# drscotthawley/signaltrain

Hardware: AMD Instinct MI355X
Metric: audio-frames/sec (train step) comp_4c 8192-sample windows @ 1/2/4/8 GPUs (higher is better)
Workload: dtype f32; 1 GPU; comp_4c synthetic, 8192-sample windows, batch 256/GPU, fp32 (BASELINE configs[1]); window=8192, frames_per_window=25, global_batch=256, parallelism=dp1

## Files before the change

### signaltrain_amd/csrc/st_ae.h

```cpp
#pragma once
#include "st_common.h"

namespace sta {

constexpr int NL = 9;
#ifndef ST_AE_ABLATE
#define ST_AE_ABLATE 0
#endif

struct AEOffsets { int w[NL]; int b[NL]; };

struct GroupWalk { int first, end, stride; };
__device__ __forceinline__ GroupWalk fwd_group_walk(const int ngroups, const int NW, const int wave)
{
    const int G = (int)gridDim.x, b = (int)blockIdx.x;
    if ((G & 7) == 0) {
        const int S = G >> 3, x = b & 7, slot = b >> 3;
        const int per = (ngroups + 7) >> 3;
        const int lo = x * per, hi = lo + per < ngroups ? lo + per : ngroups;
        return GroupWalk{lo + wave * S + slot, hi, S * NW};
    }
    return GroupWalk{wave * G + b, ngroups, G * NW};
}

// ... 108 lines not shown
                                   const int tid, const int l0, const int l1, const bool dgrad_images)
{
    const float* const nets[1] = {ae};
    ae_load_nets<NT, BF, 1>(lds, CL::tab(), nets, go, T, OT, K, tid, l0, l1, dgrad_images, true);
}
template <int NT, int BF = 0>
__device__ inline void ae_load_lds2(float* lds, const float* __restrict__ ae_m, const float* __restrict__ ae_p, const AEOffsets& go,
                                    const int T, const int OT, const int K, const int tid, const int l0, const int l1)
{
    const float* const nets[2] = {ae_m, ae_p};
    ae_load_nets<NT, BF, 2>(lds, CL::tab(), nets, go, T, OT, K, tid, l0, l1, false, true);
}

template <int NT>
__host__ __device__ __forceinline__ void ae_partials_store(float* base, const float* lds, const int stride, const AETab& tab, const AEOffsets& go,
                                                           const int PG, const int T, const int OT, const int K, const int tid, const int l0, const int l1,
                                                           const unsigned have_mask)
{
    auto sum4 = [&](int idx) { return (lds[idx] + lds[stride + idx]) + (lds[2 * stride + idx] + lds[3 * stride + idx]); };
    const AEShape sh{T, OT, K};
#pragma unroll
    for (int l = 0; l < NL; ++l) {
        if (l < l0 || l >= l1) continue;
        const bool have = (have_mask >> l) & 1;
        const int IN = sh.in(l), n = sh.out(l) * IN;
#pragma unroll
        for (int u = 0; u < (ae_max_elems(l) + NT - 1) / NT; ++u) {
            const int e = tid + u * NT;
            if (e < n) { const int o = e / IN, i = e - o * IN; base[go.w[l] + e] = have ? sum4(tab.ao[l] + o * ae_inp(l) + i) : 0.f; }
        }
        if (tid < sh.out(l)) base[go.b[l] + tid] = have ? sum4(tab.bo[l] + tid) : 0.f;
        { const int p0 = go.w[l] + n, np = go.b[l] - p0; if (tid < np) base[p0 + tid] = 0.f; }
        { const int p0 = go.b[l] + sh.out(l), np = (l + 1 < NL ? go.w[l + 1] : PG) - p0; if (tid < np) base[p0 + tid] = 0.f; }
    }
}

constexpr int AE_IMG_DG = CL::BWD_TOTAL - CL::FWD_TOTAL;
__host__ __device__ constexpr int ae_img_fwd_floats(const int FP) { return 2 * CL::FWD_TOTAL + FP; }
__host__ __device__ constexpr int ae_img_floats(const int FP) { return ae_img_fwd_floats(FP) + 2 * AE_IMG_DG; }
struct AEImgJob { const float* ae[2]; float* img; AEOffsets go; int T, OT, K, F, FP; float expfac; int n, n_blk; };
__host__ __device__ __forceinline__ float ae_freq_weight(const float expfac, const int f) { return expf(expfac * (float)f); }
__host__ __device__ __forceinline__ void ae_img_build(const AEImgJob& j, const int p)
{
    if (p >= j.n) return;
    const AEShape sh{j.T, j.OT, j.K};
    constexpr AETab tab = CL::tab();
    float v = 0.f;
    const int q0 = p - 2 * CL::FWD_TOTAL;
    if (q0 >= 0 && q0 < j.FP) v = q0 < j.F ? ae_freq_weight(j.expfac, q0) : 0.f;
    else {
        const bool dg = q0 >= 0;
        const int net = dg ? (q0 - j.FP >= AE_IMG_DG) : (p >= CL::FWD_TOTAL);
        const int q = dg ? q0 - j.FP - net * AE_IMG_DG : p - net * CL::FWD_TOTAL;
        const float* __restrict__ ae = j.ae[net];
        if (!dg && q >= CL::AEND) {
#pragma unroll
            for (int l = 0; l < NL; ++l)
                if (q >= tab.bo[l] && q < tab.bo[l] + ae_outp(l)) { const int o = q - tab.bo[l]; if (o < sh.out(l)) v = ae[j.go.b[l] + o]; }
        } else {
#pragma unroll
            for (int l = 0; l < NL; ++l)
                if (q >= tab.ao[l] && q < tab.ao[l] + ae_max_elems(l)) {
                    const int s = (q - tab.ao[l]) >> 2, lo = (q - tab.ao[l]) & 3;
                    const int o = dg ? ((s / ae_inp(l)) << 2) + lo : s % ae_outp(l);
                    const int i = dg ? s % ae_inp(l) : ((s / ae_outp(l)) << 2) + lo;
                    if (o < sh.out(l) && i < sh.in(l)) v = ae[j.go.w[l] + o * sh.in(l) + i];
// ... 577 lines not shown
#pragma unroll
        for (int it = 0; it < ITL; ++it)
#pragma unroll
            for (int r = 0; r < 4; ++r) {
                float* p = dW + (16 * ot + 4 * g + r) * INP + 16 * it + c;
                if constexpr (FIRST) *p = acc[ot][it][r]; else *p += acc[ot][it][r];
            }
}
template <int OTL, bool FIRST>
__device__ __forceinline__ void db_flush(float* dst, float (&db)[OTL], const int g, const int c)
{
#pragma unroll
    for (int ot = 0; ot < OTL; ++ot) {
        float v = db[ot];
        v += __shfl_xor(v, 16); v += __shfl_xor(v, 32);
        if (g == 0) { if constexpr (FIRST) dst[16 * ot + c] = v; else dst[16 * ot + c] += v; }
    }
}

__device__ __forceinline__ void group_colsum_store(float* __restrict__ dst, const f32x4& t, const int g, const int c)
{
    const float v = (t[0] + t[1]) + (t[2] + t[3]);
    const unsigned u = __builtin_bit_cast(unsigned, v);
    const auto p = __builtin_amdgcn_permlane16_swap(u, u, false, false);
    const float w = __builtin_bit_cast(float, (unsigned)p[0]) + __builtin_bit_cast(float, (unsigned)p[1]);
    const unsigned x = __builtin_bit_cast(unsigned, w);
    const auto q = __builtin_amdgcn_permlane32_swap(x, x, false, false);
    const float s = __builtin_bit_cast(float, (unsigned)q[0]) + __builtin_bit_cast(float, (unsigned)q[1]);
    if (g == 0) dst[c] = s;
}

constexpr int AE_BWD_SCR = (32 + 16 + 16) * SP + 2 * 4 * 320;
constexpr int ae_bwd_lds_floats(int nw) { return (CL::BWD_TOTAL + nw * AE_BWD_SCR) > nw * CL::FWD_TOTAL ? (CL::BWD_TOTAL + nw * AE_BWD_SCR) : nw * CL::FWD_TOTAL; }
template <int NW, bool INNER = false, int BF = 0, int VAR = 1, bool SAVED = false, bool KG = false, bool IMG = false>
__global__ void __launch_bounds__(NW * 64, 1)
ae_bwd_kernel(const float* __restrict__ mag, const float* __restrict__ phs, const float* __restrict__ knobs,
              const float* __restrict__ ae_m, const float* __restrict__ ae_p, const AEOffsets go, const int PG,
              const float* __restrict__ mag_hat, const float* __restrict__ phs_hat, const float* __restrict__ dAA,
              const float* __restrict__ g_mag_hat, const float reg_coef, const float expfac,
              float* __restrict__ dmag, float* __restrict__ dphs, float* __restrict__ ws,
              const int B, const int T, const int OT, const int F, const int K, const int KP,
              const int to_lo, const int to_hi,
              const int nslab, const size_t slab,
              const float* __restrict__ sv = nullptr,
              float* __restrict__ kg = nullptr,
              const float* __restrict__ img = nullptr)
{
    static_assert(!SAVED || (!INNER && BF == 0), "the kept-activation backward exists for the fused fp32 geometries");
    static_assert(!IMG || SAVED, "ready-made images: the kept-activation backward only");
    extern __shared__ __attribute__((aligned(16))) float lds[];
    const int ae = blockIdx.y;
    const int tid = threadIdx.x, lane = tid & 63, wave = tid >> 6;
    const int g = lane >> 4, c = lane & 15;
    float* lw = lds;
    float* Vs = lds + CL::BWD_TOTAL + wave * AE_BWD_SCR;
    float* Ys = Vs + 32 * SP;
    float* Ts = Ys + 16 * SP;
    float* XH = Ts + 16 * SP;
    float* XD = XH + 4 * 320;
    if constexpr (IMG && !(ST_AE_ABLATE & 128)) {
        const int FPi = KP / 2;
        const float* const dg = img + 2 * CL::FWD_TOTAL + FPi + ae * AE_IMG_DG;
        constexpr int N4 = AE_IMG_DG / 4, U = (N4 + NW * 64 - 1) / (NW * 64);
        f32x4 v[U];
#pragma unroll
        for (int u = 0; u < U; ++u) { const int e = tid + u * NW * 64; v[u] = reinterpret_cast<const f32x4*>(dg)[e < N4 ? e : 0]; }
        for (int i = tid; i < FPi / 4; i += NW * 64) reinterpret_cast<f32x4*>(lds)[i] = reinterpret_cast<const f32x4*>(img + 2 * CL::FWD_TOTAL)[i];
#pragma unroll
        for (int u = 0; u < U; ++u) { const int e = tid + u * NW * 64; if (e < N4) reinterpret_cast<f32x4*>(lds + CL::G0)[e] = v[u]; }
    } else
    ae_load_lds<NW * 64, BF>(lw, ae ? ae_p : ae_m, go, INNER ? 16 : T, INNER ? 16 : OT, K, tid, INNER ? 1 : 0, INNER ? 8 : NL, true);
    __syncthreads();

    const float* vin = ae ? phs : mag;
    const float* dh8in = ae ? phs_hat : mag_hat;
    float* dvout = ae ? dphs : dmag;
    const int FP = KP / 2, gpw = FP / 16;
    const int ngroups = B * gpw;
    const int gstride = gridDim.x * NW;

    f32x4 rW1[4][2], rW2[2][4], rW3[1][2], rW4[1][1], rW5[1][2], rW6[1][1], rW7[2][1], rW8[4][2], rW9[1][4];
    float rb1[4], rb2[2], rb3[1], rb4[1], rb5[1], rb6[1], rb7[2], rb8[4], rb9[1];
// ... 52 lines not shown
        const float* const dB0 = dA0 + FP, * const dB1 = dA1 + FP, * const dB2 = dA2 + FP;
        const unsigned bOT = ST_MUL24(bq, OT), btF = ST_MUL24(ST_MUL24(bq, T), F) + (unsigned)fq;
#pragma unroll
        for (int r = 0; r < 4; ++r) {
            const int to = 4 * g + r;
            const bool ok = fvq && to < OT;
            const bool lv = ok && to >= to_lo && to <= to_hi;
            const unsigned ro = bOT + (unsigned)(ok ? to : 0);
            const unsigned p0 = ST_MUL24(lv ? ro : 0u, KP) + (unsigned)fq;
            const unsigned pF = ST_MUL24(ro, F) + (unsigned)fq;
#if ST_AE_ABLATE & 1
            q_x[r][0] = q_x[r][1] = q_x[r][2] = q_y[r][0] = q_y[r][1] = q_y[r][2] = 1e-3f * (float)(p0 & 7); q_ph[r] = 0.3f; q_mh[r] = 0.2f + 1e-3f * (float)(pF & 3);
#else
            q_x[r][0] = ldg32(dA0, p0); q_x[r][1] = ldg32(dA1, p0); q_x[r][2] = ldg32(dA2, p0);
            q_y[r][0] = ldg32(dB0, p0); q_y[r][1] = ldg32(dB1, p0); q_y[r][2] = ldg32(dB2, p0);
            q_ph[r] = ldg32(phs_hat, pF); q_mh[r] = ldg32(mag_hat, pF);
#endif
            if constexpr (GM) q_gm[r] = ldg32(g_mag_hat, pF); else q_gm[r] = 0.f;
            if constexpr (!TAIL16) q_mt[r] = ldg32(vin, btF + ST_MUL24(ok ? T - OT + to : 0, F));
        }
    };
    f32x4 s_h1[4], s_h2[2], s_h3[1], s_h4[1], s_h5[1], s_h6[1], s_h7[2], s_h8[4], s_e9[1];
    const float* const svn = SAVED ? sv + (size_t)ae * ngroups * (AE_SV_TILES * 256) : nullptr;
    const unsigned lane16 = (unsigned)lane << 4;
#ifdef ST_SV_DIAG
    auto svp = [&](const int gq) { return svn + (size_t)(__builtin_amdgcn_readfirstlane(gq) & ST_SV_DIAG) * (AE_SV_TILES * 256); };
#else
    auto svp = [&](const int gq) { return svn + (size_t)__builtin_amdgcn_readfirstlane(gq) * (AE_SV_TILES * 256); };
#endif
    if constexpr (SAVED) {
        if (grp < ngroups) {
            load_q(grp);
            const float* const p = svp(grp);
            sv_load(p, lane16, 16, s_e9); sv_load(p, lane16, 12, s_h8); sv_load(p, lane16, 10, s_h7); sv_load(p, lane16, 9, s_h6); sv_load(p, lane16, 8, s_h5);
            sv_load(p, lane16, 7, s_h4); sv_load(p, lane16, 6, s_h3); sv_load(p, lane16, 4, s_h2); sv_load(p, lane16, 0, s_h1);
        }
    }

    for (; grp < ngroups; grp += gstride) {
        asm volatile("" ::: "memory");
        const int b = grp / gpw, f = (grp - b * gpw) * 16 + c;
        const bool fv = f < F;
        if constexpr (!INNER && !SAVED) load_q(grp);
        f32x4 h1in[4], dh8[4];
        if constexpr (INNER) {
            const unsigned col0 = (unsigned)b * FP + (unsigned)(grp - b * gpw) * 16;
#pragma unroll
            for (int ot = 0; ot < 4; ++ot) {
#pragma unroll
                for (int r = 0; r < 4; ++r) {
                    h1in[ot][r] = ldg32(vin, (unsigned)(16 * ot + 4 * g + r) * Rw + col0 + c);
                    dh8[ot][r] = ldg32(dh8in, (unsigned)(16 * ot + 4 * g + r) * Rw + col0 + c);
                }
            }
        }
        f32x4 vn[2], knn; float knTn;
        const int gnext = grp + gstride < ngroups ? grp + gstride : grp;
#if ST_AE_ABLATE & 64
        vn[0] = vr[0]; vn[1] = vr[1]; knn = kn; knTn = knT;
#else
        if constexpr (!INNER) load_v(gnext, vn);
        load_kn(gnext, knn, knTn);
#endif

        f32x4 h1[4], h2[2], h3[1], h4[1], h5[1], h6[1], h7[2], h8[4], e9[1];
        f32x4 fr9[1 * 4];
        if constexpr (SAVED) {
#pragma unroll
            for (int it = 0; it < 2; ++it)
#pragma unroll
                for (int r = 0; r < 4; ++r) Vs[(16 * it + 4 * g + r) * SP + c] = vr[it][r];
#pragma unroll
            for (int k = 0; k < 4; ++k) { h1[k] = s_h1[k]; h8[k] = s_h8[k]; }
#pragma unroll
            for (int k = 0; k < 2; ++k) { h2[k] = s_h2[k]; h7[k] = s_h7[k]; }
            h3[0] = s_h3[0]; h4[0] = s_h4[0]; h5[0] = s_h5[0]; h6[0] = s_h6[0]; e9[0] = s_e9[0];
        } else {
        f32x4 fr2[2 * 4];
        if constexpr (INNER) {
#pragma unroll
            for (int ot = 0; ot < 4; ++ot) h1[ot] = h1in[ot];
            frags_fwd<2, 4, CL::O1, BF>(fr2, lw + CL::A1, g, c);
        } else {
            f32x4 fr1[4 * 2]; frags_fwd<4, 2, CL::O0, BF>(fr1, lw + CL::A0, g, c);
            frags_fwd<2, 4, CL::O1, BF>(fr2, lw + CL::A1, g, c);
#pragma unroll
            for (int it = 0; it < 2; ++it)
#pragma unroll
                for (int r = 0; r < 4; ++r) Vs[(16 * it + 4 * g + r) * SP + c] = vr[it][r];
            ST_FENCE();
            fwdD_fr<4, 2, BF>(fr1, lw + CL::B0, vr, h1, g);
        }
        f32x4 fr3[1 * 2]; frags_fwd<1, 2, CL::O2, BF>(fr3, lw + CL::A2, g, c); ST_FENCE(); fwdD_fr<2, 4, BF>(fr2, lw + CL::B1, h1, h2, g);
        f32x4 fr4[1 * 1]; frags_fwd<1, 1, CL::O3, BF>(fr4, lw + CL::A3, g, c); ST_FENCE(); fwdD_fr<1, 2, BF>(fr3, lw + CL::B2, h2, h3, g);
        f32x4 fr5[1 * 2]; frags_fwd<1, 2, CL::O4, BF>(fr5, lw + CL::A4, g, c); ST_FENCE(); fwdD_fr<1, 1, BF>(fr4, lw + CL::B3, h3, h4, g);
        f32x4 fr6[1 * 1]; frags_fwd<1, 1, CL::O5, BF>(fr6, lw + CL::A5, g, c); ST_FENCE();
        {
            const f32x4 hk[2] = {h4[0], kn};
            fwdD_fr<1, 2, BF>(fr5, lw + CL::B4, hk, h5, g);
        }
        f32x4 fr7[2 * 1]; frags_fwd<2, 1, CL::O6, BF>(fr7, lw + CL::A6, g, c); ST_FENCE(); fwdD_fr<1, 1, BF>(fr6, lw + CL::B5, h5, h6, g);
        f32x4 fr8[4 * 2]; frags_fwd<4, 2, CL::O7, BF>(fr8, lw + CL::A7, g, c); ST_FENCE(); fwdD_fr<2, 1, BF>(fr7, lw + CL::B6, h6, h7, g);
        if constexpr (!INNER) frags_fwd<1, 4, CL::O8, BF>(fr9, lw + CL::A8, g, c);
        ST_FENCE(); fwdD_fr<4, 2, BF>(fr8, lw + CL::B7, h7, h8, g);
        }
        f32x4 da9[1];
        float dxA[4], mtA[4];
        if constexpr (!INNER) {
            ST_FENCE();
// ... 6 lines not shown
                const bool ok = fv && to < OT;
                const bool lv = ok && to >= to_lo && to <= to_hi;
                const float gre = lv ? q_x[r][0] + (nslab > 1 ? q_x[r][1] : 0.f) + (nslab > 2 ? q_x[r][2] : 0.f) : 0.f;
                const float gim = lv ? q_y[r][0] + (nslab > 1 ? q_y[r][1] : 0.f) + (nslab > 2 ? q_y[r][2] : 0.f) : 0.f;
                const float ph = q_ph[r], mh = q_mh[r];
                if constexpr (!TAIL16) asm volatile("" :: "v"(q_mt[r]));
                float sn, cs; st_sincos(ph, sn, cs);
                const float sg = mh > 0.f ? 1.f : (mh < 0.f ? -1.f : 0.f);
                const float dmh = gre * cs + gim * sn + reg_coef * sg * wf + (GM ? q_gm[r] : 0.f);
                const float dph = mh * (gim * cs - gre * sn);
                dxA[r] = ok ? (ae == 0 ? dmh : dph) : 0.f;
                mtA[r] = ae == 0 ? (TAIL16 ? vr[1][r] : q_mt[r]) : 1.f;
            }
            if constexpr (!SAVED) fwdD_fr<1, 4, BF>(fr9, lw + CL::B8, h8, e9, g);
            if constexpr (BF == 0 && !SAVED) {
#pragma unroll
                for (int p_ = 0; p_ < 16; ++p_) { __builtin_amdgcn_sched_group_barrier(0x008, 1, 0); __builtin_amdgcn_sched_group_barrier(0x002, 7, 0); }
            }
            ST_FENCE();
        }
        if constexpr (!INNER) {
#pragma unroll
            for (int r = 0; r < 4; ++r) {
                const int to = 4 * g + r;
                const float eg = elu_grad_from_out(e9[0][r]);
                const float e1 = ae == 0 ? e9[0][r] : 1.f;
                const float d9 = dxA[r] * mtA[r] * eg;
                const float tail = dxA[r] * e1;
                da9[0][r] = d9;
                Ts[to * SP + c] = tail;
                Ys[to * SP + c] = d9;
            }
        }
#define ST_REFILL(...) do { if constexpr (SAVED) { ST_FENCE(); __VA_ARGS__; ST_FENCE(); } } while (0)
        const float* const svq = SAVED ? svp(gnext) : nullptr;
        ST_REFILL(load_q(gnext); sv_load(svq, lane16, 16, s_e9));
#define ST_PIPE(N_) do { \
        __builtin_amdgcn_sched_group_barrier(0x008, (N_) + 2, 0); \
        _Pragma("unroll") for (int p_ = 0; p_ < (N_) - 2; ++p_) { \
            __builtin_amdgcn_sched_group_barrier(0x002, 2, 0); __builtin_amdgcn_sched_group_barrier(0x300, 1, 0); \
            __builtin_amdgcn_sched_group_barrier(0x008, 1, 0); } \
        ST_FENCE(); } while (0)
#define ST_BWD_STAGE(O_, I_, FD_, DA_, DAT_, HP_, HTP_, DAP_, DATP_, RW_, RB_, NEXT_) \
        to_Th<I_, BF>(XH, HP_, HTP_, g, c); ST_FENCE(); \
        dgradD_fr<O_, I_, BF>(FD_, DA_, DAP_); mul_elu_grad<I_>(DAP_, HP_); \
        to_T<I_>(XD, DAP_, DATP_, g, c); NEXT_; \
        wgrad_regh<O_, I_, BF>(RW_, RB_, DAT_, HTP_); \
        ST_PIPE(BF ? O_ * I_ : O_ * I_ * 4);
        typedef typename TTy<BF>::type tt_t;
        tt_t hT8[4]; f32x4 da8[4], daT8[4], fd8[2 * 4];
        if constexpr (INNER) {
            frags_dgrad<4, 2, CL::I7, BF>(fd8, lw + CL::G7, g, c);
            to_Th<4, BF>(XH, h8, hT8, g, c);
#pragma unroll
            for (int ot = 0; ot < 4; ++ot) da8[ot] = dh8[ot];
            mul_elu_grad<4>(da8, h8); to_T<4>(XD, da8, daT8, g, c);
        } else {
            f32x4 daT9[1], fd9[4 * 1];
            frags_dgrad<1, 4, CL::I8, BF>(fd9, lw + CL::G8, g, c);
            daT9[0] = *reinterpret_cast<const f32x4*>(Ys + c * SP + 4 * g);
            ST_BWD_STAGE(1, 4, fd9, da9, daT9, h8, hT8, da8, daT8, rW9, rb9, (frags_dgrad<4, 2, CL::I7, BF>(fd8, lw + CL::G7, g, c)))
            ST_REFILL(sv_load(svq, lane16, 12, s_h8));
        }
        tt_t hT7[2]; f32x4 da7[2], daT7[2], fd7[1 * 2];
        ST_BWD_STAGE(4, 2, fd8, da8, daT8, h7, hT7, da7, daT7, rW8, rb8, (frags_dgrad<2, 1, CL::I6, BF>(fd7, lw + CL::G6, g, c)))
        ST_REFILL(sv_load(svq, lane16, 10, s_h7));
        tt_t hT6[1]; f32x4 da6[1], daT6[1], fd6[1];
        ST_BWD_STAGE(2, 1, fd7, da7, daT7, h6, hT6, da6, daT6, rW7, rb7, (frags_dgrad<1, 1, CL::I5, BF>(fd6, lw + CL::G5, g, c)))
        ST_REFILL(sv_load(svq, lane16, 9, s_h6));
        tt_t hT5[1]; f32x4 da5[1], daT5[1], fd5[1];
        ST_BWD_STAGE(1, 1, fd6, da6, daT6, h5, hT5, da5, daT5, rW6, rb6, (frags_dgrad<1, 1, CL::I4, BF>(fd5, lw + CL::G4, g, c)))
        ST_REFILL(sv_load(svq, lane16, 8, s_h5));
        tt_t hT4[1], hT4k[2]; f32x4 da4[1], daT4[1], fd4[1];
        {
            to_Th<1, BF>(XH, h4, hT4, g, c); ST_FENCE();
            dgradD_fr<1, 1, BF>(fd5, da5, da4); mul_elu_grad<1>(da4, h4);
            to_T<1>(XD, da4, daT4, g, c); frags_dgrad<1, 1, CL::I3, BF>(fd4, lw + CL::G3, g, c); ST_FENCE();
            hT4k[0] = hT4[0];
            hT4k[1] = tt_splat<BF>(knT);
            wgrad_regh<1, 2, BF>(rW5, rb5, daT5, hT4k);
            if constexpr (KG) group_colsum_store(kg + ((size_t)ae * ngroups + grp) * 16, daT5[0], g, c);
        }
        ST_REFILL(sv_load(svq, lane16, 7, s_h4));
        tt_t hT3[1]; f32x4 da3[1], daT3[1], fd3[2 * 1];
        ST_BWD_STAGE(1, 1, fd4, da4, daT4, h3, hT3, da3, daT3, rW4, rb4, (frags_dgrad<1, 2, CL::I2, BF>(fd3, lw + CL::G2, g, c)))
        ST_REFILL(sv_load(svq, lane16, 6, s_h3));
        tt_t hT2[2]; f32x4 da2[2], daT2[2], fd2[4 * 2];
        ST_BWD_STAGE(1, 2, fd3, da3, daT3, h2, hT2, da2, daT2, rW3, rb3, (frags_dgrad<2, 4, CL::I1, BF>(fd2, lw + CL::G1, g, c)))
        ST_REFILL(sv_load(svq, lane16, 4, s_h2));
        tt_t hT1[4]; f32x4 da1[4], daT1[4], fd1[2 * 4];
        if constexpr (INNER) {
            to_Th<4, BF>(XH, h1, hT1, g, c); ST_FENCE();
            dgradD_fr<2, 4, BF>(fd2, da2, da1); mul_elu_grad<4>(da1, h1);
            const unsigned col0 = (unsigned)b * FP + (unsigned)(grp - b * gpw) * 16;
#pragma unroll
            for (int ot = 0; ot < 4; ++ot)
#pragma unroll
                for (int r = 0; r < 4; ++r) stg32(dvout, (unsigned)(16 * ot + 4 * g + r) * Rw + col0 + c, da1[ot][r]);
            ST_FENCE();
            wgrad_regh<2, 4, BF>(rW2, rb2, daT2, hT1);
        } else {
            ST_BWD_STAGE(2, 4, fd2, da2, daT2, h1, hT1, da1, daT1, rW2, rb2, (frags_dgrad<4, 2, CL::I0, BF>(fd1, lw + CL::G0, g, c)))
            ST_REFILL(sv_load(svq, lane16, 0, s_h1));
        }
        f32x4 vT[2], dv[2];
        if constexpr (!INNER) {
#pragma unroll
            for (int it = 0; it < 2; ++it) vT[it] = *reinterpret_cast<const f32x4*>(Vs + (16 * it + c) * SP + 4 * g);
            ST_FENCE();
            dgradD_fr<4, 2, BF>(fd1, da1, dv);
            wgrad_reg<4, 2, BF>(rW1, rb1, daT1, vT);
        }
#undef ST_BWD_STAGE
#undef ST_PIPE
#undef ST_REFILL
        if constexpr (!INNER) {
            mask_v(gnext, vn);
            vr[0] = vn[0]; vr[1] = vn[1];
        }
        mask_kn(knn, knTn); kn = knn; knT = knTn;
        if constexpr (!INNER) {
        float dvs[2][4], tls[2][4];
#pragma unroll
        for (int it = 0; it < 2; ++it)
#pragma unroll
            for (int r = 0; r < 4; ++r) {
                dvs[it][r] = dv[it][r]; asm volatile("" : "+v"(dvs[it][r]));
                const int ti = 16 * it + 4 * g + r - (T - OT);
                tls[it][r] = Ts[(ti >= 0 && ti < OT ? ti : 0) * SP + c];
            }
        const unsigned dv0 = ST_MUL24(ST_MUL24(b, T), F) + (unsigned)f;
#pragma unroll
        for (int it = 0; it < 2; ++it)
#pragma unroll
            for (int r = 0; r < 4; ++r) {
                const int t = 16 * it + 4 * g + r;
                const float v = dvs[it][r] + (t >= T - OT ? tls[it][r] : 0.f);
#if ST_AE_ABLATE & 2
                asm volatile("" :: "v"(v));
#else
                if (fv && t < T) stg32(dvout, dv0 + ST_MUL24(t, F), v);
#endif
            }
        }
    }
#if ST_AE_ABLATE & 256
    {
#define ST_KT(x, A, Bq) { _Pragma("unroll") for (int a_ = 0; a_ < A; ++a_) _Pragma("unroll") for (int b_ = 0; b_ < Bq; ++b_) _Pragma("unroll") for (int r_ = 0; r_ < 4; ++r_) asm volatile("" :: "v"(x[a_][b_][r_])); }
#define ST_KB(x, A) { _Pragma("unroll") for (int a_ = 0; a_ < A; ++a_) asm volatile("" :: "v"(x[a_])); }
        ST_KT(rW1, 4, 2) ST_KT(rW2, 2, 4) ST_KT(rW3, 1, 2) ST_KT(rW4, 1, 1) ST_KT(rW5, 1, 2) ST_KT(rW6, 1, 1) ST_KT(rW7, 2, 1) ST_KT(rW8, 4, 2) ST_KT(rW9, 1, 4)
        ST_KB(rb1, 4) ST_KB(rb2, 2) ST_KB(rb3, 1) ST_KB(rb4, 1) ST_KB(rb5, 1) ST_KB(rb6, 1) ST_KB(rb7, 2) ST_KB(rb8, 4) ST_KB(rb9, 1)
#undef ST_KT
#undef ST_KB
        return;
    }
#endif
    __syncthreads();
    static_assert(NW == 4, "the store pass sums exactly four per-wave images");
    float* dwl = lds + wave * CL::FWD_TOTAL;
    if constexpr (!INNER) { dw_flush<4, 2, CL::I0, true>(dwl + CL::A0, rW1, g, c); dw_flush<1, 4, CL::I8, true>(dwl + CL::A8, rW9, g, c);
                            db_flush<4, true>(dwl + CL::B0, rb1, g, c); db_flush<1, true>(dwl + CL::B8, rb9, g, c); }
    dw_flush<2, 4, CL::I1, true>(dwl + CL::A1, rW2, g, c); dw_flush<1, 2, CL::I2, true>(dwl + CL::A2, rW3, g, c);
    dw_flush<1, 1, CL::I3, true>(dwl + CL::A3, rW4, g, c); dw_flush<1, 2, CL::I4, true>(dwl + CL::A4, rW5, g, c);
    dw_flush<1, 1, CL::I5, true>(dwl + CL::A5, rW6, g, c); dw_flush<2, 1, CL::I6, true>(dwl + CL::A6, rW7, g, c);
    dw_flush<4, 2, CL::I7, true>(dwl + CL::A7, rW8, g, c);
    db_flush<2, true>(dwl + CL::B1, rb2, g, c); db_flush<1, true>(dwl + CL::B2, rb3, g, c); db_flush<1, true>(dwl + CL::B3, rb4, g, c);
    db_flush<1, true>(dwl + CL::B4, rb5, g, c); db_flush<1, true>(dwl + CL::B5, rb6, g, c); db_flush<2, true>(dwl + CL::B6, rb7, g, c);
    db_flush<4, true>(dwl + CL::B7, rb8, g, c);
    __syncthreads();
    ae_partials_store<NW * 64>(ws + ((size_t)blockIdx.x * 2 + ae) * PG, lds, CL::FWD_TOTAL, CL::tab(), go, PG, T, OT, K, tid, 0, NL,
                               INNER ? 0x0FEu : 0x1FFu);
}

}
```

### signaltrain_amd/csrc/st_api.hip

```cpp
#include <hip/hip_runtime.h>
#include <stdarg.h>
#include <stdio.h>
#include <string.h>
#include <math.h>
#include <mutex>
#include <set>
#include <type_traits>
#include <utility>
#include "st_common.h"
#include "st_gemm.h"
#include "st_gemm_planes.h"
#include "st_gemm_tn.h"
#include "st_gemm16.h"
#include "st_misc.h"
#include "st_ae.h"
#include "st_ae_wide.h"
#include "st_ae_split.h"
#include "st_ae32.h"
#include "st_dp.h"
#include "st_feed.h"
#include "st_feed_files.h"

static thread_local char g_err[512] = "";
int st_fail(int code, const char* fmt, ...)
// ... 132 lines not shown
    return n;
}
extern "C" int st_set_debug(int v) { return v == 0 ? ST_OK : st_fail(ST_ERR_ARG, "st_set_debug(%d): the product library has no run-time ablations (build with -DST_*_ABLATE=bits)", v); }
static int g_dp_inline = 1;
static int g_ae_save = 1;
static int g_ae_split = -1;
static int g_ae32 = 1;
static int g_pl_bf16 = 0;
static int g_wg_split = 0;
static int g_pl_dgrad = 0;
static int g_pl_shape = 3;
static int g_g16 = 1;
static int g_g16_dma = 0;
static int g_nt128 = 1;
static int g_tn128 = 1;
static int g_tn_fm = 3;
static int g_g16_crop = 15;
static int g_frs_nt = 1;
static int g_xt = 0;
static const int NORM_E_PARTIALS = 32;
static const int NORM_E_MAX = 4096;
static int g_wide_direct = 1;
static int g_an_bk = 32;
static int g_bk = 16;
static int g_wg_mode = 0;
#define ST_TUNING_LIST(X) X(g_ae_split, -1) X(g_ae_save, 1) X(g_dp_inline, 1) X(g_pl_bf16, 0) X(g_wg_split, 0) X(g_pl_dgrad, 0) X(g_pl_shape, 3) X(g_g16, 1) X(g_g16_dma, 0) \
    X(g_nt128, 1) X(g_tn128, 1) X(g_frs_nt, 1) X(g_xt, 0) X(g_an_bk, 32) X(g_bk, 16) X(g_wg_mode, 0) X(g_ae32, 1) X(g_wide_direct, 1) X(g_tn_fm, 3) X(g_g16_crop, 15)
static const struct { int first, count; int* var; int value; int* also; } k_tuning_codes[] = {
    {16, 1, &g_an_bk, 16, &g_bk}, {32, 1, &g_an_bk, 32, &g_bk},
    {100, 1, &g_wg_mode, 0, nullptr}, {102, 1, &g_wg_mode, 2, nullptr},
    {7000, 2, &g_xt, 0, nullptr},
    {8000, 2, &g_ae_split, 0, nullptr}, {8002, 1, &g_ae_split, -1, nullptr},
    {8100, 2, &g_ae32, 0, nullptr},
    {8200, 3, &g_ae_save, 0, nullptr},
    {8300, 2, &g_dp_inline, 0, nullptr},
    {9000, 2, &g_frs_nt, 0, nullptr},
    {9100, 1, &g_pl_shape, 0, nullptr}, {9103, 1, &g_pl_shape, 3, nullptr},
    {9200, 2, &g_pl_dgrad, 0, nullptr},
    {9300, 2, &g_wg_split, 0, nullptr},
    {9400, 2, &g_pl_bf16, 0, nullptr},
    {9500, 2, &g_tn128, 0, nullptr}, {9580, 1, &g_tn128, 2, nullptr}, {9581, 1, &g_tn128, 1, nullptr},
    {9540, 4, &g_tn_fm, 0, nullptr},
    {9560, 16, &g_g16_crop, 0, nullptr},
    {9600, 2, &g_g16, 0, nullptr},
    {9690, 4, &g_g16_dma, 0, nullptr},
    {9950, 2, &g_nt128, 0, nullptr},
    {9970, 2, &g_wide_direct, 0, nullptr},
};
extern "C" int st_set_tuning(int code)
{
    for (const auto& t : k_tuning_codes)
        if (code >= t.first && code < t.first + t.count) { *t.var = t.value + (code - t.first); if (t.also) *t.also = *t.var; return ST_OK; }
    return st_fail(ST_ERR_ARG, "st_set_tuning(%d): no such code", code);
}
extern "C" int st_get_tuning(int* out, int n)
{
    int i = 0;
#define X(v_, d_) if (out && i < n) out[i] = v_; ++i;
    ST_TUNING_LIST(X)
#undef X
    return i;
}
extern "C" int st_tuning_defaults(int* out, int n)
{
    int i = 0;
#define X(v_, d_) if (out && i < n) out[i] = d_; ++i;
    ST_TUNING_LIST(X)
// ... 18 lines not shown
                              else if (ht_ == 3) { ST_TRY((stg::launch_half<W_, 1, 3>(__VA_ARGS__))); } \
                              else if (g_xt) { if ((BK_) == 16) stg::launch<W_, 16, true>(__VA_ARGS__); else stg::launch<W_, 32, true>(__VA_ARGS__); } \
                              else if ((BK_) == 16) stg::launch<W_, 16>(__VA_ARGS__); else stg::launch<W_, 32>(__VA_ARGS__); } while (0)
#define ST_GEMM(W_, ...) ST_GEMM_BK(g_bk, W_, __VA_ARGS__)
#define ST_GEMM_AN(W_, ...) ST_GEMM_BK(g_an_bk, W_, __VA_ARGS__)
#define ST_GEMM_WG(...) do { if (g_wg_mode == 2 && gemm_ht(d->prec) == 0) stg::launch<3, 16, true>(__VA_ARGS__); \
                             else if (gemm_ht(d->prec) == 3 && !g_wg_split) stg::launch<3, 16>(__VA_ARGS__); else ST_GEMM(3, __VA_ARGS__); } while (0)
static int ensure_dyn_lds(const void* fn, const char* name)
{
    static std::mutex mu; static std::set<std::pair<int, const void*>> done;
    int dev = 0; (void)hipGetDevice(&dev);
    std::lock_guard<std::mutex> lk(mu);
    if (done.count({dev, fn})) return ST_OK;
    const hipError_t e = hipFuncSetAttribute(fn, hipFuncAttributeMaxDynamicSharedMemorySize, 160 * 1024);
    if (e != hipSuccess) return st_fail(ST_ERR_LAUNCH, "hipFuncSetAttribute(%s, 160 KB dynamic LDS): %s", name, hipGetErrorString(e));
    done.insert({dev, fn});
    return ST_OK;
}
template <class... P, class... A>
static int launch_lds(const char* name, void (*kernel)(P...), dim3 grid, dim3 block, size_t lds, hipStream_t s, A&&... args)
{
    static_assert(sizeof...(P) == sizeof...(A), "launch_lds: argument count");
    ST_TRY(ensure_dyn_lds(reinterpret_cast<const void*>(kernel), name));
    hipLaunchKernelGGL(kernel, grid, block, lds, s, static_cast<P>(args)...);
    return ST_OK;
}
template <int V> using ic = std::integral_constant<int, V>;
template <class F> static inline auto with_ht(int ht, F&& f) { return ht == 1 ? f(ic<1>{}) : ht == 2 ? f(ic<2>{}) : f(ic<0>{}); }
template <class F> static inline auto with_ht16(int ht, F&& f) { return ht == 2 ? f(ic<2>{}) : f(ic<1>{}); }
template <class F> static inline auto with_bool(bool b, F&& f) { return b ? f(std::true_type{}) : f(std::false_type{}); }
template <class F> static inline auto with_var(int var, F&& f) { return with_ht(var, f); }
template <class F> static inline auto with_slabs(int ns, F&& f) { return ns == 3 ? f(ic<3>{}) : ns == 2 ? f(ic<2>{}) : f(ic<1>{}); }
static const int AE_FWD_NW = 8, AE_BWD_NW = 4;
template <class F> static inline auto with_fwd_nw(int nw, F&& f) { return nw == 11 ? f(ic<11>{}) : f(ic<AE_FWD_NW>{}); }
template <class F> static inline auto with_inner_nw(int nw, F&& f) { return nw == 9 ? f(ic<9>{}) : nw == 12 ? f(ic<12>{}) : f(ic<AE_FWD_NW>{}); }
static int synth_live_rows(const st_dims* d);
static bool ae_is_wide(const st_dims* d);
static int ae_fwd_groups(const st_dims* d) { return d->B * (st_kp_of(d->F) / 32); }
static int ae_fwd_nw(const st_dims* d)
{
    if (ae_is_wide(d) || ae_ht(d->prec) != 0) return AE_FWD_NW;
    const int groups = ae_fwd_groups(d), c = num_cus();
    auto cost = [&](int nw) { int grid = (groups + nw - 1) / nw; if (grid > c) grid = c; const int rounds = (groups + grid * nw - 1) / (grid * nw); return rounds * nw; };
    return cost(11) < cost(AE_FWD_NW) ? 11 : AE_FWD_NW;
}
static int ae_inner_nw(const st_dims* d)
{
    const int groups = ae_fwd_groups(d), c = num_cus();
    int best = AE_FWD_NW, best_cost = 1 << 30;
    for (int nw : {8, 9, 12}) {
        int grid = (groups + nw - 1) / nw; if (grid > c) grid = c;
        const int rounds = (groups + grid * nw - 1) / (grid * nw), cost = rounds * ((nw + 3) / 4);
        if (cost < best_cost) { best_cost = cost; best = nw; }
    }
    return best;
}
static int ae_inner_grid(const st_dims* d) { const int nw = ae_inner_nw(d); int g = (ae_fwd_groups(d) + nw - 1) / nw; int c = num_cus(); return g < c ? g : c; }
static int ae_fwd_grid(const st_dims* d) { const int nw = ae_fwd_nw(d); int g = (ae_fwd_groups(d) + nw - 1) / nw; int c = num_cus(); return g < c ? g : c; }
static int ae_bwd_grid(const st_dims* d) { int groups = d->B * (st_kp_of(d->F) / 32); int g = (groups + AE_BWD_NW - 1) / AE_BWD_NW; int c = num_cus() / 2; if (c < 1) c = 1; return g < c ? g : c; }
static const int WSPLIT_ROWS = 200, WSPLIT_MAX = 16;
static int wgrad_split(int R) { int s = R / WSPLIT_ROWS; if (s < 1) s = 1; if (s > WSPLIT_MAX) s = WSPLIT_MAX; return s; }
static int wgrad_split_tiles(int R, int M, int Nc)
{
    int s = wgrad_split(R);
    const int tiles = ((M + 95) / 96) * ((Nc + 95) / 96), slots = 6 * num_cus();
    int fit = slots / (tiles > 0 ? tiles : 1); if (fit < 1) fit = 1;
// ... 578 lines not shown
    const stg::RowMap live = synth_live(d);
    const int t_hi = live.t_lo + live.Tv - 1, nsl = synth_slabs(d);
    const size_t slab = (size_t)d->B * d->OT * L.KP;
    hipStream_t s = st_stream(stream);
    float* h4x = ws;
    float* da4x = ws + ae_h4_floats(d);
    float* parts = ws + 2 * ae_h4_floats(d);
    int grid = ae_bwd_grid(d);
    const int ht = ae_ht(d->prec);
    if (ae_use_split(d)) {
        if (!have_fwd)
            ST_TRY(ae_fwd_body(d, L, mag, phs, knobs, ae_m, ae_p, nullptr, nullptr, nullptr, nullptr, h4x, stream));
        grid = ae_split_grid(d);
        static_assert((size_t)sta::ae_split_lds_floats<1>(AE_SPLIT_NW) * sizeof(float) <= 160 * 1024 && (size_t)sta::ae_split_lds_floats<2>(AE_SPLIT_NW) * sizeof(float) <= 160 * 1024, "split ae_bwd LDS budget");
        auto part = [&](auto PART, auto HT, auto GM, auto KG) {
            return launch_lds("ae_bwd_part_kernel", sta::ae_bwd_part_kernel<AE_SPLIT_NW, PART(), HT(), GM(), KG()>, dim3(grid, 2), dim3(AE_SPLIT_NW * 64),
                              (size_t)sta::ae_split_lds_floats<PART()>(AE_SPLIT_NW) * sizeof(float), s,
                              mag, phs, knobs, ae_m, ae_p, L.go, L.PG, mag_hat, phs_hat, dAA, g_mag_hat, reg_coef, expfac, dmag, dphs, parts,
                              h4x, da4x, d->B, d->T, d->OT, d->F, d->K, L.KP, live.t_lo, t_hi, nsl, slab, kg); };
        auto halves = [&](auto HT, auto KG) -> int {
            ST_TRY(with_bool(g_mag_hat != nullptr, [&](auto GM) { return part(ic<1>{}, HT, GM, KG); }));
            ST_LAUNCHED("ae_bwd_dec");
            ST_TRY(part(ic<2>{}, HT, std::false_type{}, std::false_type{}));
            ST_LAUNCHED("ae_bwd_enc");
            return ST_OK; };
        if (kg) ST_TRY(with_ht16(ht, [&](auto HT) { return halves(HT, std::true_type{}); }));
        else ST_TRY(with_ht(ht, [&](auto HT) { return halves(HT, std::false_type{}); }));
    } else {
        const int var = g_mag_hat ? 1 : (d->T - d->OT == 16 ? 2 : 0);
        if (have_fwd && ae_use_saved(d)) {
            const float* sv = ae_sv_ptr(d, L, ws);
            const float* img = (have_img && ae_img_level(d) == 2) ? ae_img_ptr(ws) : nullptr;
            ST_TRY(with_var(var, [&](auto VAR) { return with_bool(kg != nullptr, [&](auto KG) { return with_bool(img != nullptr, [&](auto IMG) {
                return launch_lds("ae_bwd_kernel", sta::ae_bwd_kernel<AE_BWD_NW, false, 0, VAR(), true, KG(), IMG()>, dim3(grid, 2), dim3(AE_BWD_NW * 64), lds, s,
                                  mag, phs, knobs, ae_m, ae_p, L.go, L.PG, mag_hat, phs_hat, dAA, g_mag_hat, reg_coef, expfac,
                                  dmag, dphs, parts, d->B, d->T, d->OT, d->F, d->K, L.KP, live.t_lo, t_hi, nsl, slab, sv, kg, img); }); }); }));
        } else
            ST_TRY(with_ht(ht, [&](auto HT) { return with_var(var, [&](auto VAR) {
                return launch_lds("ae_bwd_kernel", sta::ae_bwd_kernel<AE_BWD_NW, false, HT(), VAR()>, dim3(grid, 2), dim3(AE_BWD_NW * 64), lds, s,
                                  mag, phs, knobs, ae_m, ae_p, L.go, L.PG, mag_hat, phs_hat, dAA, g_mag_hat, reg_coef, expfac,
                                  dmag, dphs, parts, d->B, d->T, d->OT, d->F, d->K, L.KP, live.t_lo, t_hi, nsl, slab, nullptr, nullptr, nullptr); }); }));
        ST_LAUNCHED("ae_bwd");
    }
    if (defer_reduce && *defer_reduce) return ST_OK;
    hipLaunchKernelGGL(stm::ae_grad_reduce_kernel, dim3((L.PG + 63) / 64, 2), dim3(256), 0, s, parts, grid, L.PG, g_m, g_p);
    ST_LAUNCHED("ae_grad_reduce"); return ST_OK;
}
extern "C" int st_ae_bwd(const st_dims* d, const float* mag, const float* phs, const float* knobs,
                         const float* ae_m, const float* ae_p, const float* mag_hat, const float* phs_hat,
                         const float* dAA, const float* g_mag_hat, float reg_coef, float* dmag, float* dphs, float* ws,
                         float* g_m, float* g_p, void* stream)
{
    Layout L; ST_TRY(make_layout(d, &L));
    return ae_bwd_body(d, L, mag, phs, knobs, ae_m, ae_p, mag_hat, phs_hat, dAA, g_mag_hat, reg_coef, dmag, dphs, ws, g_m, g_p, false, stream);
}

extern "C" int st_polar_bwd(const st_dims* d, const float* re, const float* im, const float* dmag, const float* dphs,
                            const float* g_mag, float* dG, void* stream)
{
    ST_TRY(check_dims(d)); ST_REQ(re && im && dmag && dphs && dG, "st_polar_bwd: null pointer");
    const int R = d->B * d->T, KP = st_kp_of(d->F);
    hipLaunchKernelGGL(stm::polar_bwd_kernel, dim3((KP / 2 + 255) / 256, R), dim3(256), 0, st_stream(stream),
                       re, im, dmag, dphs, g_mag, dG, R, d->F, KP, gemm_ht(d->prec) == 2 ? 65504.0f : 0.0f);
    ST_LAUNCHED("polar_bwd"); return ST_OK;
}

static int analysis_wgrad_impl(const st_dims* d, const float* dG, const float* sig, bool padded, float in_scale, float* ws,
                               float* gWr, float* gWi, float* norm_partial, void* stream, int half = -1, float* stage = nullptr, int stage_bf16 = 0)
{
// ... 1198 lines not shown
        const int np = norm_partials(d);
        hipLaunchKernelGGL(stm::unstage_l1_kernel, dim3(2 * d->F), dim3(256), 0, st_stream(stream), stage, grads + L.offs[0], grads + L.offs[1], d->F, d->N, gs, w.norm_a, np, pack16);
        ST_LAUNCHED("unstage_l1");
        stm::FinArgs f = fin_args(d, w.loss_p, w.reg_p, w.norm_a, w.norm_s, 1.0f);
        if (d->clip_all) { f.norm_e = w.norm_e; f.n_ne = NORM_E_PARTIALS; }
        return clip_adam_impl(params, grads, m, v, L.total, d->clip_all ? L.total : L.n_stft, scalars, gs, lr, beta1, beta2, eps, step, &f, stream);
    }
}


struct st_graph { hipGraph_t graph; hipGraphExec_t exec; };

static int attr_prepare(const st_dims* d)
{
    auto prep = [](auto* kernel, const char* name) { return ensure_dyn_lds(reinterpret_cast<const void*>(kernel), name); };
    const int ht = ae_ht(d->prec);
    if (ae_is_wide(d))
        ST_TRY(with_ht(ht, [&](auto HT) -> int {
            ST_TRY(prep(sta::ae_inner_fwd_kernel<AE_FWD_NW, HT()>, "ae_inner_fwd_kernel")); ST_TRY(prep(sta::ae_inner_fwd_kernel<9, HT()>, "ae_inner_fwd_kernel"));
            ST_TRY(prep(sta::ae_inner_fwd_kernel<12, HT()>, "ae_inner_fwd_kernel"));
            ST_TRY(prep(sta::ae_bwd_kernel<AE_BWD_NW, true, HT(), 0>, "ae_bwd_kernel"));
            return prep(stw::wide_dv_polar_kernel<HT()>, "wide_dv_polar_kernel"); }));
    else {
        ST_TRY(with_ht(ht, [&](auto HT) -> int {
            ST_TRY(prep(sta::ae_fwd_kernel<AE_FWD_NW, HT()>, "ae_fwd_kernel"));
            ST_TRY(prep(sta::ae_bwd_part_kernel<AE_SPLIT_NW, 1, HT(), false>, "ae_bwd_part_kernel")); ST_TRY(prep(sta::ae_bwd_part_kernel<AE_SPLIT_NW, 2, HT(), false>, "ae_bwd_part_kernel"));
            return d->T - d->OT == 16 ? prep(sta::ae_bwd_kernel<AE_BWD_NW, false, HT(), 2>, "ae_bwd_kernel") : prep(sta::ae_bwd_kernel<AE_BWD_NW, false, HT(), 0>, "ae_bwd_kernel"); }));
        if (ht != 0) ST_TRY(with_ht16(ht, [&](auto HT) { return prep(sta::ae_fwd32_kernel<AE_FWD_NW, HT()>, "ae_fwd32_kernel"); }));
        else {
            ST_TRY(prep(sta::ae_fwd_kernel<11, 0>, "ae_fwd_kernel")); ST_TRY(prep(sta::ae_fwd_kernel<11, 0, true>, "ae_fwd_kernel")); ST_TRY(prep(sta::ae_fwd_kernel<AE_FWD_NW, 0, true>, "ae_fwd_kernel"));
            for (int var = 0; var < 3; ++var)
                ST_TRY(with_var(var, [&](auto VAR) -> int {
                    ST_TRY(prep(sta::ae_bwd_kernel<AE_BWD_NW, false, 0, VAR(), true>, "ae_bwd_kernel"));
                    return prep(sta::ae_bwd_kernel<AE_BWD_NW, false, 0, VAR(), true, false, true>, "ae_bwd_kernel"); }));
        }
    }
    if (g_nt128 && gemm_ht(d->prec) == 0) ST_TRY(prep(stg::gemm_nt128_kernel, "gemm_nt128_kernel"));
    if (use_g16(d))
        ST_TRY(with_ht16(gemm_ht(d->prec), [&](auto HT) -> int {
            ST_TRY(prep(stg::gemm16_nt256_kernel<HT(), stg::PolarStore>, "gemm16_nt256_kernel")); ST_TRY(prep(stg::gemm16_nt256_kernel<HT(), stg::StoreC>, "gemm16_nt256_kernel"));
            ST_TRY(prep(stg::gemm16_nt_kernel<HT(), 64, stg::PolarStore>, "gemm16_nt_kernel")); ST_TRY(prep(stg::gemm16_nt_kernel<HT(), 64, stg::StoreC>, "gemm16_nt_kernel"));
            return prep(stg::gemm16_tn_kernel<HT(), 64>, "gemm16_tn_kernel"); }));
    if (use_planes(d)) {
        ST_TRY(prep(stg::gemm_planes_kernel<4, 3, stg::FramedNT<true>, stg::ChunkP, stg::PolarStore>, "gemm_planes_kernel"));
        ST_TRY(prep(stg::gemm_planes_kernel<8, 3, stg::FramedNT<true>, stg::ChunkP, stg::PolarStore>, "gemm_planes_kernel"));
        ST_TRY(prep(stg::gemm_planes_kernel<4, 3, stg::PlainNT, stg::ChunkP, stg::StoreC>, "gemm_planes_kernel"));
        ST_TRY(prep(stg::gemm_planes_kernel<4, 3, stg::FramedNT<true>, stg::ChunkP, stg::StoreC>, "gemm_planes_kernel"));
    }
    (void)num_cus();
    return ST_OK;
}

extern "C" int st_graph_create(const st_dims* d, float* params, float* grads, float* m, float* v, const float* x,
                               const float* knobs, const float* y_true, void* ws, float* scalars,
                               const float* lr_table, int n_lr, float beta1, float beta2, float eps, void* stream, st_graph** out)
{
    ST_TRY(check_dims(d));
    ST_REQ(params && grads && m && v && x && (knobs || d->K == 0) && y_true && ws && scalars && lr_table && n_lr > 0 && out, "st_graph_create: bad arguments");
    ST_REQ(!g_prof, "st_graph_create: switch the event profiling off first (event records would be captured)");
    ST_TRY(attr_prepare(d));
    hipStream_t s = st_stream(stream);
    if (hipStreamBeginCapture(s, hipStreamCaptureModeThreadLocal) != hipSuccess) return st_fail(ST_ERR_LAUNCH, "st_graph_create: hipStreamBeginCapture failed (is `stream` the legacy default stream?)");
    hipLaunchKernelGGL(stm::step_tick_kernel, dim3(1), dim3(64), 0, s, scalars, lr_table, n_lr);
    int rc = train_step_impl(d, params, grads, m, v, x, knobs, y_true, ws, scalars, 0.f, beta1, beta2, eps, 1, stream, true);
    hipGraph_t g = nullptr;
    const hipError_t e = hipStreamEndCapture(s, &g);
    if (rc != ST_OK) { if (g) (void)hipGraphDestroy(g); return rc; }
// ... 23 lines not shown
```

Before: 11.16 million frames/s.

## Trim saved-activation register lifetimes and vectorize partial-gradient stores in AE backward

Adds two options to the saved-activation autoencoder backward kernel. The NEAR option stops keeping every prefetched hidden activation in registers across iterations. It loads the middle layers at the start of each group and the first layers just before use, and moves the next-group prefetch later. This cuts register pressure but gives less time to hide load latency. The WTAIL option writes the per-block weight and bias partial sums with 16-byte vector loads and stores when the pointers are aligned, replacing scalar element stores. Both are enabled by default through ST_AE_TRIM=3 unless the g_ae_save setting equals 3.

```diff
diff --git a/signaltrain_amd/csrc/st_ae.h b/signaltrain_amd/csrc/st_ae.h
--- a/signaltrain_amd/csrc/st_ae.h
+++ b/signaltrain_amd/csrc/st_ae.h
@@ -164,6 +164,53 @@
         if (tid < sh.out(l)) base[go.b[l] + tid] = have ? sum4(tab.bo[l] + tid) : 0.f;
         { const int p0 = go.w[l] + n, np = go.b[l] - p0; if (tid < np) base[p0 + tid] = 0.f; }
         { const int p0 = go.b[l] + sh.out(l), np = (l + 1 < NL ? go.w[l + 1] : PG) - p0; if (tid < np) base[p0 + tid] = 0.f; }
+    }
+}
+
+template <int NT>
+__host__ __device__ __forceinline__ void ae_partials_store_wide(float* base, const float* lds, const int stride, const AETab& tab, const AEOffsets& go,
+                                                                const int PG, const int T, const int OT, const int K, const int tid, const int l0, const int l1,
+                                                                const unsigned have_mask)
+{
+    auto sum4 = [&](int idx) {
+        const f32x4 a = *reinterpret_cast<const f32x4*>(lds + idx), b = *reinterpret_cast<const f32x4*>(lds + stride + idx);
+        const f32x4 c = *reinterpret_cast<const f32x4*>(lds + 2 * stride + idx), d = *reinterpret_cast<const f32x4*>(lds + 3 * stride + idx);
+        return (a + b) + (c + d);
+    };
+    auto put = [&](const int at, const f32x4 v, const int n, const bool wide) {
+        if (wide && n >= 4) *reinterpret_cast<f32x4*>(base + at) = v;
+        else {
+#pragma unroll
+            for (int k = 0; k < 4; ++k) if (k < n) base[at + k] = v[k];
+        }
+    };
+    const AEShape sh{T, OT, K};
+    const bool al16 = (reinterpret_cast<size_t>(base) & 15) == 0;
+#pragma unroll
+    for (int l = 0; l < NL; ++l) {
+        if (l < l0 || l >= l1) continue;
+        const bool have = (have_mask >> l) & 1;
+        const int IN = sh.in(l), OUT = sh.out(l), n = OUT * IN;
+        const int ip = ae_inp(l), q = ip >> 2, ns = ae_outp(l) * q;
+        const bool wide_w = al16 && ((go.w[l] | IN) & 3) == 0;
+#pragma unroll
+        for (int u = 0; u < (ae_max_elems(l) / 4 + NT - 1) / NT; ++u) {
+            const int s = tid + u * NT;
+            const int o = s / q, i = (s - o * q) << 2;
+            if (s < ns && o < OUT && i < IN) {
+                const f32x4 v = have ? sum4(tab.ao[l] + o * ip + i) : (f32x4){0.f, 0.f, 0.f, 0.f};
+                put(go.w[l] + o * IN + i, v, IN - i, wide_w);
+            }
+        }
+        {
+            const int t = tid - (l % (NT / 64)) * 64, o = t * 4;
+            if (t >= 0 && o < OUT) {
+                const f32x4 v = have ? sum4(tab.bo[l] + o) : (f32x4){0.f, 0.f, 0.f, 0.f};
+                put(go.b[l] + o, v, OUT - o, al16 && (go.b[l] & 3) == 0);
+            }
+        }
+        { const int p0 = go.w[l] + n, np = go.b[l] - p0; if (tid < np) base[p0 + tid] = 0.f; }
+        { const int p0 = go.b[l] + OUT, np = (l + 1 < NL ? go.w[l + 1] : PG) - p0; if (tid < np) base[p0 + tid] = 0.f; }
     }
 }
 
@@ -807,7 +854,7 @@
 
 constexpr int AE_BWD_SCR = (32 + 16 + 16) * SP + 2 * 4 * 320;
 constexpr int ae_bwd_lds_floats(int nw) { return (CL::BWD_TOTAL + nw * AE_BWD_SCR) > nw * CL::FWD_TOTAL ? (CL::BWD_TOTAL + nw * AE_BWD_SCR) : nw * CL::FWD_TOTAL; }
-template <int NW, bool INNER = false, int BF = 0, int VAR = 1, bool SAVED = false, bool KG = false, bool IMG = false>
+template <int NW, bool INNER = false, int BF = 0, int VAR = 1, bool SAVED = false, bool KG = false, bool IMG = false, bool WTAIL = false, bool NEAR = false>
 __global__ void __launch_bounds__(NW * 64, 1)
 ae_bwd_kernel(const float* __restrict__ mag, const float* __restrict__ phs, const float* __restrict__ knobs,
               const float* __restrict__ ae_m, const float* __restrict__ ae_p, const AEOffsets go, const int PG,
@@ -823,6 +870,7 @@
 {
     static_assert(!SAVED || (!INNER && BF == 0), "the kept-activation backward exists for the fused fp32 geometries");
     static_assert(!IMG || SAVED, "ready-made images: the kept-activation backward only");
+    static_assert((!WTAIL && !NEAR) || SAVED, "the 16-byte store pass and the near refills: the kept-activation backward only");
     extern __shared__ __attribute__((aligned(16))) float lds[];
     const int ae = blockIdx.y;
     const int tid = threadIdx.x, lane = tid & 63, wave = tid >> 6;
@@ -941,8 +989,9 @@
         if (grp < ngroups) {
             load_q(grp);
             const float* const p = svp(grp);
-            sv_load(p, lane16, 16, s_e9); sv_load(p, lane16, 12, s_h8); sv_load(p, lane16, 10, s_h7); sv_load(p, lane16, 9, s_h6); sv_load(p, lane16, 8, s_h5);
-            sv_load(p, lane16, 7, s_h4); sv_load(p, lane16, 6, s_h3); sv_load(p, lane16, 4, s_h2); sv_load(p, lane16, 0, s_h1);
+            sv_load(p, lane16, 16, s_e9); sv_load(p, lane16, 12, s_h8); sv_load(p, lane16, 10, s_h7);
+            if constexpr (!NEAR) { sv_load(p, lane16, 9, s_h6); sv_load(p, lane16, 8, s_h5);
+                                   sv_load(p, lane16, 7, s_h4); sv_load(p, lane16, 6, s_h3); sv_load(p, lane16, 4, s_h2); sv_load(p, lane16, 0, s_h1); }
         }
     }
 
@@ -974,16 +1023,26 @@
 
         f32x4 h1[4], h2[2], h3[1], h4[1], h5[1], h6[1], h7[2], h8[4], e9[1];
         f32x4 fr9[1 * 4];
+        const float* const svc = SAVED && NEAR ? svp(grp) : nullptr;
         if constexpr (SAVED) {
 #pragma unroll
             for (int it = 0; it < 2; ++it)
 #pragma unroll
                 for (int r = 0; r < 4; ++r) Vs[(16 * it + 4 * g + r) * SP + c] = vr[it][r];
+            if constexpr (NEAR) {
+#pragma unroll
+                for (int k = 0; k < 4; ++k) h8[k] = s_h8[k];
+#pragma unroll
+                for (int k = 0; k < 2; ++k) h7[k] = s_h7[k];
+                e9[0] = s_e9[0];
+                sv_load(svc, lane16, 9, h6); sv_load(svc, lane16, 8, h5); sv_load(svc, lane16, 7, h4); sv_load(svc, lane16, 6, h3);
+            } else {
 #pragma unroll
             for (int k = 0; k < 4; ++k) { h1[k] = s_h1[k]; h8[k] = s_h8[k]; }
 #pragma unroll
             for (int k = 0; k < 2; ++k) { h2[k] = s_h2[k]; h7[k] = s_h7[k]; }
             h3[0] = s_h3[0]; h4[0] = s_h4[0]; h5[0] = s_h5[0]; h6[0] = s_h6[0]; e9[0] = s_e9[0];
+            }
         } else {
         f32x4 fr2[2 * 4];
         if constexpr (INNER) {
@@ -1056,7 +1115,8 @@
                 Ys[to * SP + c] = d9;
             }
         }
-#define ST_REFILL(...) do { if constexpr (SAVED) { ST_FENCE(); __VA_ARGS__; ST_FENCE(); } } while (0)
+#define ST_REFILL(...) do { if constexpr (SAVED && !NEAR) { ST_FENCE(); __VA_ARGS__; ST_FENCE(); } } while (0)
+#define ST_REFILL_NEAR(...) do { if constexpr (SAVED && NEAR) { ST_FENCE(); __VA_ARGS__; ST_FENCE(); } } while (0)
         const float* const svq = SAVED ? svp(gnext) : nullptr;
         ST_REFILL(load_q(gnext); sv_load(svq, lane16, 16, s_e9));
 #define ST_PIPE(N_) do { \
@@ -1085,6 +1145,7 @@
             daT9[0] = *reinterpret_cast<const f32x4*>(Ys + c * SP + 4 * g);
             ST_BWD_STAGE(1, 4, fd9, da9, daT9, h8, hT8, da8, daT8, rW9, rb9, (frags_dgrad<4, 2, CL::I7, BF>(fd8, lw + CL::G7, g, c)))
             ST_REFILL(sv_load(svq, lane16, 12, s_h8));
+            ST_REFILL_NEAR(sv_load(svc, lane16, 4, h2); sv_load(svc, lane16, 0, h1));
         }
         tt_t hT7[2]; f32x4 da7[2], daT7[2], fd7[1 * 2];
         ST_BWD_STAGE(4, 2, fd8, da8, daT8, h7, hT7, da7, daT7, rW8, rb8, (frags_dgrad<2, 1, CL::I6, BF>(fd7, lw + CL::G6, g, c)))
@@ -1112,6 +1173,7 @@
         tt_t hT2[2]; f32x4 da2[2], daT2[2], fd2[4 * 2];
         ST_BWD_STAGE(1, 2, fd3, da3, daT3, h2, hT2, da2, daT2, rW3, rb3, (frags_dgrad<2, 4, CL::I1, BF>(fd2, lw + CL::G1, g, c)))
         ST_REFILL(sv_load(svq, lane16, 4, s_h2));
+        ST_REFILL_NEAR(load_q(gnext); sv_load(svq, lane16, 16, s_e9); sv_load(svq, lane16, 12, s_h8); sv_load(svq, lane16, 10, s_h7));
         tt_t hT1[4]; f32x4 da1[4], daT1[4], fd1[2 * 4];
         if constexpr (INNER) {
             to_Th<4, BF>(XH, h1, hT1, g, c); ST_FENCE();
@@ -1138,6 +1200,7 @@
 #undef ST_BWD_STAGE
 #undef ST_PIPE
 #undef ST_REFILL
+#undef ST_REFILL_NEAR
         if constexpr (!INNER) {
             mask_v(gnext, vn);
             vr[0] = vn[0]; vr[1] = vn[1];
@@ -1192,6 +1255,8 @@
     db_flush<1, true>(dwl + CL::B4, rb5, g, c); db_flush<1, true>(dwl + CL::B5, rb6, g, c); db_flush<2, true>(dwl + CL::B6, rb7, g, c);
     db_flush<4, true>(dwl + CL::B7, rb8, g, c);
     __syncthreads();
+    if constexpr (WTAIL) ae_partials_store_wide<NW * 64>(ws + ((size_t)blockIdx.x * 2 + ae) * PG, lds, CL::FWD_TOTAL, CL::tab(), go, PG, T, OT, K, tid, 0, NL, 0x1FFu);
+    else
     ae_partials_store<NW * 64>(ws + ((size_t)blockIdx.x * 2 + ae) * PG, lds, CL::FWD_TOTAL, CL::tab(), go, PG, T, OT, K, tid, 0, NL,
                                INNER ? 0x0FEu : 0x1FFu);
 }
diff --git a/signaltrain_amd/csrc/st_api.hip b/signaltrain_amd/csrc/st_api.hip
--- a/signaltrain_amd/csrc/st_api.hip
+++ b/signaltrain_amd/csrc/st_api.hip
@@ -188,7 +188,7 @@
     {7000, 2, &g_xt, 0, nullptr},
     {8000, 2, &g_ae_split, 0, nullptr}, {8002, 1, &g_ae_split, -1, nullptr},
     {8100, 2, &g_ae32, 0, nullptr},
-    {8200, 3, &g_ae_save, 0, nullptr},
+    {8200, 4, &g_ae_save, 0, nullptr},
     {8300, 2, &g_dp_inline, 0, nullptr},
     {9000, 2, &g_frs_nt, 0, nullptr},
     {9100, 1, &g_pl_shape, 0, nullptr}, {9103, 1, &g_pl_shape, 3, nullptr},
@@ -273,6 +273,10 @@
 template <class F> static inline auto with_var(int var, F&& f) { return with_ht(var, f); }
 template <class F> static inline auto with_slabs(int ns, F&& f) { return ns == 3 ? f(ic<3>{}) : ns == 2 ? f(ic<2>{}) : f(ic<1>{}); }
 static const int AE_FWD_NW = 8, AE_BWD_NW = 4;
+#ifndef ST_AE_TRIM
+#define ST_AE_TRIM 3
+#endif
+static constexpr bool AE_TRIM(bool on, int bit) { return on && (ST_AE_TRIM & bit) != 0; }
 template <class F> static inline auto with_fwd_nw(int nw, F&& f) { return nw == 11 ? f(ic<11>{}) : f(ic<AE_FWD_NW>{}); }
 template <class F> static inline auto with_inner_nw(int nw, F&& f) { return nw == 9 ? f(ic<9>{}) : nw == 12 ? f(ic<12>{}) : f(ic<AE_FWD_NW>{}); }
 static int synth_live_rows(const st_dims* d);
@@ -917,9 +921,11 @@
             const float* sv = ae_sv_ptr(d, L, ws);
             const float* img = (have_img && ae_img_level(d) == 2) ? ae_img_ptr(ws) : nullptr;
             ST_TRY(with_var(var, [&](auto VAR) { return with_bool(kg != nullptr, [&](auto KG) { return with_bool(img != nullptr, [&](auto IMG) {
-                return launch_lds("ae_bwd_kernel", sta::ae_bwd_kernel<AE_BWD_NW, false, 0, VAR(), true, KG(), IMG()>, dim3(grid, 2), dim3(AE_BWD_NW * 64), lds, s,
+                return with_bool(g_ae_save != 3, [&](auto TRIM) {
+                return launch_lds("ae_bwd_kernel", sta::ae_bwd_kernel<AE_BWD_NW, false, 0, VAR(), true, KG(), IMG(), AE_TRIM(TRIM(), 1), AE_TRIM(TRIM(), 2)>,
+                                  dim3(grid, 2), dim3(AE_BWD_NW * 64), lds, s,
                                   mag, phs, knobs, ae_m, ae_p, L.go, L.PG, mag_hat, phs_hat, dAA, g_mag_hat, reg_coef, expfac,
-                                  dmag, dphs, parts, d->B, d->T, d->OT, d->F, d->K, L.KP, live.t_lo, t_hi, nsl, slab, sv, kg, img); }); }); }));
+                                  dmag, dphs, parts, d->B, d->T, d->OT, d->F, d->K, L.KP, live.t_lo, t_hi, nsl, slab, sv, kg, img); }); }); }); }));
         } else
             ST_TRY(with_ht(ht, [&](auto HT) { return with_var(var, [&](auto VAR) {
                 return launch_lds("ae_bwd_kernel", sta::ae_bwd_kernel<AE_BWD_NW, false, HT(), VAR()>, dim3(grid, 2), dim3(AE_BWD_NW * 64), lds, s,
@@ -2184,7 +2190,9 @@
             for (int var = 0; var < 3; ++var)
                 ST_TRY(with_var(var, [&](auto VAR) -> int {
                     ST_TRY(prep(sta::ae_bwd_kernel<AE_BWD_NW, false, 0, VAR(), true>, "ae_bwd_kernel"));
-                    return prep(sta::ae_bwd_kernel<AE_BWD_NW, false, 0, VAR(), true, false, true>, "ae_bwd_kernel"); }));
+                    ST_TRY(prep(sta::ae_bwd_kernel<AE_BWD_NW, false, 0, VAR(), true, false, true>, "ae_bwd_kernel"));
+                    ST_TRY(prep(sta::ae_bwd_kernel<AE_BWD_NW, false, 0, VAR(), true, false, false, AE_TRIM(true, 1), AE_TRIM(true, 2)>, "ae_bwd_kernel"));
+                    return prep(sta::ae_bwd_kernel<AE_BWD_NW, false, 0, VAR(), true, false, true, AE_TRIM(true, 1), AE_TRIM(true, 2)>, "ae_bwd_kernel"); }));
         }
     }
     if (g_nt128 && gemm_ht(d->prec) == 0) ST_TRY(prep(stg::gemm_nt128_kernel, "gemm_nt128_kernel"));
```

Result: no change. 11.16 million frames/s (median of 2 runs) (+0.0%).
